# apache/datafusion

Hardware: AMD Instinct MI355X
Metric: tpch_q3_hash_join_rows_per_sec (higher is better)
Workload: dtype int64 keys / decimal128 payload; 1 GPU; INNER hash-join orders⋈lineitem on o_orderkey, TPC-H SF100, Q3 payload (o_orderdate,o_shippriority,l_orderkey,l_extendedprice,l_discount), device-resident inputs; build_rows=150000000, probe_rows=599960064, output_rows=599960064, join_table=rank_map, probe=single_pass_unordered, parallelism=single GPU, exchange=none

## Files before the change

datafusion_amd/csrc/internal.hpp:

```cpp
#pragma once
#include <atomic>
#include <hip/hip_runtime.h>

#include <chrono>
#include <cstdint>
#include <cstring>
#include <map>
#include <memory>
#include <mutex>
#include <stdexcept>
#include <string>
#include <thread>
#include <vector>

#include "../../include/dfgpu.h"

namespace dfgpu {

struct Error : std::runtime_error {
  using std::runtime_error::runtime_error;
};

void set_last_error(const std::string& msg);

// ... 79 lines not shown

  bool profiling = false;
  struct Rec {
    std::string name;
    hipEvent_t a, b;
    int64_t bytes;
    std::thread::id thread;
  };
  std::map<std::thread::id, int64_t> kernel_ns_by_thread;
  std::vector<Rec> recs;
  std::vector<dfgpu_kernel_stat> stats;
  struct Launch { int stat; float ms; int64_t bytes; };
  std::vector<Launch> launches;
  void collect();
};

Runtime& rt();
void scan_upload_caches_drop(int device);
int64_t scan_upload_caches_bytes(int device);
Runtime& rt_of(int device);
void use_device(int device);
int current_device();
const std::vector<int>& initialised_devices();
void require_init();

struct ProfileScope {
  hipEvent_t a = nullptr, b = nullptr;
  const char* name;
  int64_t bytes;
  ProfileScope(const char* name, int64_t algorithmic_bytes);
  ~ProfileScope();
};

struct DevBuf {
  void* ptr = nullptr;
  size_t bytes = 0;
  Runtime* owner = nullptr;
  std::shared_ptr<void> foreign;
  std::atomic<uint64_t> hint{0};
  std::atomic<uint64_t> all_hit_hint{0};
  explicit DevBuf(size_t n);
  DevBuf(void* p, size_t n, std::shared_ptr<void> keep_alive) : ptr(p), bytes(n), foreign(std::move(keep_alive)) {}
  ~DevBuf();
  DevBuf(const DevBuf&) = delete;
  DevBuf& operator=(const DevBuf&) = delete;
  template <typename T>
  T* as() const { return reinterpret_cast<T*>(ptr); }
};
using BufPtr = std::shared_ptr<DevBuf>;
inline BufPtr make_buf(size_t bytes) { return std::make_shared<DevBuf>(bytes ? bytes : 1); }
BufPtr make_zero_buf(size_t bytes);

void d2h(void* dst, const void* src, size_t n);
extern std::atomic<int64_t> g_pinned_driver_allocs, g_pinned_driver_ns;
void* pinned_alloc(size_t n);
void pinned_release(void* p);
void* stage_alloc(size_t n);
template <class T> struct StageAllocator {
  using value_type = T;
  StageAllocator() = default;
  template <class U> StageAllocator(const StageAllocator<U>&) {}
  T* allocate(size_t n) { return static_cast<T*>(stage_alloc(n * sizeof(T))); }
  void deallocate(T* p, size_t) { pinned_release(p); }
  template <class U> void construct(U* p) noexcept { ::new ((void*)p) U; }
  template <class U, class... A> void construct(U* p, A&&... a) { ::new ((void*)p) U(std::forward<A>(a)...); }
  template <class U> bool operator==(const StageAllocator<U>&) const { return true; }
  template <class U> bool operator!=(const StageAllocator<U>&) const { return false; }
};
template <class T> using StageVec = std::vector<T, StageAllocator<T>>;
struct PinnedBuf {
  void* ptr = nullptr;
  size_t bytes = 0;
  explicit PinnedBuf(size_t n) : ptr(pinned_alloc(n ? n : 1)), bytes(n) {}
  ~PinnedBuf() { pinned_release(ptr); }
  PinnedBuf(const PinnedBuf&) = delete;
  PinnedBuf& operator=(const PinnedBuf&) = delete;
  template <class T> T* as() const { return reinterpret_cast<T*>(ptr); }
};
void h2d_async(void* dst, const void* src, size_t n);

inline int type_width(int t) {
  switch (t) {
    case DFGPU_INT32: case DFGPU_UINT32: case DFGPU_DATE32: return 4;
    case DFGPU_INT64: case DFGPU_UINT64: case DFGPU_FLOAT64: return 8;
    case DFGPU_DECIMAL128: return 16;
    case DFGPU_UINT8: return 1;
    case DFGPU_BOOL: return 0;
    case DFGPU_UTF8:
      throw Error("a Utf8 column reached an operator that works on fixed-width columns: dictionary-encode it first (dfgpu_table_dictionary_encode)");
  }
  throw Error("unknown dfgpu_type " + std::to_string(t));
}
inline size_t bitmap_bytes(int64_t n) { return (size_t)((n + 63) / 64) * 8; }
inline size_t data_bytes(int t, int64_t n) { return t == DFGPU_BOOL ? bitmap_bytes(n) : (size_t)n * type_width(t); }
inline bool is_integer_like(int t) {
  return t == DFGPU_INT32 || t == DFGPU_INT64 || t == DFGPU_UINT8 || t == DFGPU_UINT32 || t == DFGPU_UINT64 || t == DFGPU_DATE32;
}
inline bool is_signed_type(int t) { return t == DFGPU_INT32 || t == DFGPU_INT64 || t == DFGPU_DATE32 || t == DFGPU_DECIMAL128; }
std::string type_name(const dfgpu_field& f);

struct ColStats {
  long long min = 0, max = 0;
  int64_t valid = 0;
  bool ascending = false;
  bool nondecreasing = false;
  bool has_present = false;
// ... 144 lines not shown
```

datafusion_amd/csrc/join.hip:

```cpp
#include <thread>
#include <functional>
#include <cstdlib>

#include "device.hpp"
#include "internal.hpp"
#include "grouped.hpp"

namespace dfgpu {

Table compact_table(const Table& in, const std::vector<int>& cols, const uint64_t* mask, const uint64_t* mask_valid);
void pack_bytes_to_bitmap(const uint8_t* bytes, int64_t n, uint64_t* words);

enum TableKind : int { KIND_HASH = 0, KIND_ARRAY = 1, KIND_RANK = 2, KIND_RADIX = 3, KIND_FLAT = 4, KIND_FLAT16 = 5,
                       KIND_RETURNED = 6 };
template <int KIND> constexpr bool kind_is_flat() { return KIND == KIND_FLAT || KIND == KIND_FLAT16; }
template <int KIND> constexpr bool kind_is_direct() { return KIND == KIND_ARRAY || KIND == KIND_RANK; }

struct FlatLayout {
  int n;
  uint8_t off[MAX_KEYS];
  uint8_t width[MAX_KEYS];
  int8_t null_bit[MAX_KEYS];
};
constexpr double RANK_MAP_MIN_KEY_DENSITY = 1.0 / 256.0;
// ... 253 lines not shown
      }
    }
    return;
  }
  const int64_t stride = (int64_t)gridDim.x * BLOCK;
  for (int64_t i0 = (int64_t)blockIdx.x * BLOCK + threadIdx.x; i0 < n; i0 += stride * BUILD_UNROLL) {
    uint64_t lo[BUILD_UNROLL];
    bool ok[BUILD_UNROLL];
#pragma unroll
    for (int j = 0; j < BUILD_UNROLL; j++) {
      int64_t i = i0 + j * stride;
      lo[j] = load_key<KT>(k, i < n ? i : n - 1);
    }
#pragma unroll
    for (int j = 0; j < BUILD_UNROLL; j++) {
      int64_t i = i0 + j * stride;
      ok[j] = i < n;
      if (HASV) ok[j] = ok[j] && bit_at(k.valid, i < n ? i : n - 1);
    }
#pragma unroll
    for (int j = 0; j < BUILD_UNROLL; j++) {
      if (!ok[j]) continue;
      const uint64_t idx = lo[j] - offset;
      const unsigned long long bit = 1ull << (idx & 63);
      (void)__hip_atomic_fetch_or(&bits[idx >> 6], bit, __ATOMIC_RELAXED, __HIP_MEMORY_SCOPE_AGENT);
    }
  }
}
typedef unsigned long long rt_u64x2 __attribute__((ext_vector_type(2)));
typedef unsigned rt_u32x4 __attribute__((ext_vector_type(4)));
template <int KT>
__device__ __forceinline__ void load_keys4(const KeyCol& k, int64_t i0, uint64_t (&out)[4]) {
  if (KT == KT_I64 && ((uintptr_t)k.data & 15) == 0) {
    const rt_u64x2* p = reinterpret_cast<const rt_u64x2*>((const uint64_t*)k.data + i0);
    const rt_u64x2 a = __builtin_nontemporal_load(p), b = __builtin_nontemporal_load(p + 1);
    out[0] = a.x; out[1] = a.y; out[2] = b.x; out[3] = b.y;
  } else if ((KT == KT_I32 || KT == KT_U32) && ((uintptr_t)k.data & 15) == 0) {
    const rt_u32x4 a = __builtin_nontemporal_load(reinterpret_cast<const rt_u32x4*>((const uint32_t*)k.data + i0));
    out[0] = KT == KT_I32 ? (uint64_t)(int64_t)(int32_t)a.x : a.x;
    out[1] = KT == KT_I32 ? (uint64_t)(int64_t)(int32_t)a.y : a.y;
    out[2] = KT == KT_I32 ? (uint64_t)(int64_t)(int32_t)a.z : a.z;
    out[3] = KT == KT_I32 ? (uint64_t)(int64_t)(int32_t)a.w : a.w;
  } else {
#pragma unroll
    for (int j = 0; j < 4; j++) out[j] = load_key<KT, true>(k, i0 + j);
  }
}
constexpr int RT_ROWS = 4096;
constexpr int RT_WIN = 1024;
constexpr int RT_LANE_ROWS = 4;
constexpr int RT_CHUNK = WAVE * RT_LANE_ROWS;
constexpr int RT_STEPS = RT_ROWS / RT_CHUNK / (BLOCK / WAVE);
template <int KT, bool VERIFY>
__global__ __launch_bounds__(BLOCK) void k_rank_tab_onepass(KeyCol k, int64_t n, uint64_t offset, uint64_t range, ulonglong2* __restrict__ tab, int* __restrict__ flag) {
  __shared__ unsigned long long s_bits[RT_WIN];
  __shared__ unsigned s_first[RT_WIN];
  constexpr int WAVES = BLOCK / WAVE;
  const unsigned lane = lane_id();
  const int wv = threadIdx.x >> 6;
  const int64_t r0 = (int64_t)blockIdx.x * RT_ROWS;
  const int64_t r1 = r0 + RT_ROWS < n ? r0 + RT_ROWS : n;
  const uint64_t n_words = (range >> 6) + 1;
  uint64_t idx[RT_STEPS][RT_LANE_ROWS], pidx[RT_STEPS];
#pragma unroll
  for (int c = 0; c < RT_STEPS; c++) {
    const int64_t i0 = r0 + (int64_t)(c * WAVES + wv) * RT_CHUNK + lane * RT_LANE_ROWS;
    if (i0 + RT_LANE_ROWS <= n) {
      load_keys4<KT>(k, i0, idx[c]);
#pragma unroll
      for (int j = 0; j < RT_LANE_ROWS; j++) idx[c][j] -= offset;
    } else {
#pragma unroll
      for (int j = 0; j < RT_LANE_ROWS; j++) idx[c][j] = load_key<KT, true>(k, i0 + j < n ? i0 + j : n - 1) - offset;
    }
    pidx[c] = 0;
    if (VERIFY) pidx[c] = load_key<KT>(k, i0 < n ? (i0 > 0 ? i0 - 1 : 0) : n - 1) - offset;
  }
  const bool tail_lane = wv == WAVES - 1 && r1 + lane < n;
  const uint64_t tail_idx = tail_lane ? load_key<KT>(k, r1 + lane) - offset : ~0ull;
  const uint64_t w_first = r0 > 0 ? ((load_key<KT>(k, r0 - 1) - offset) >> 6) + 1 : 0ull;
  const uint64_t w_last = (load_key<KT>(k, r1 - 1) - offset) >> 6;
  const uint64_t w_end = w_last < n_words ? w_last : n_words - 1;
  const int cnt = w_end < w_first ? 0 : (w_end - w_first + 1 < (uint64_t)RT_WIN ? (int)(w_end - w_first + 1) : RT_WIN);
  for (int t = threadIdx.x; t < cnt; t += BLOCK) {
    s_bits[t] = 0ull;
    s_first[t] = ~0u;
  }
  __syncthreads();
  auto put = [&](uint64_t w, unsigned long long bits, int64_t row, bool first_known, bool is_first) {
    const uint64_t slot = w - w_first;
    if (slot < (uint64_t)cnt) {
      atomicOr(&s_bits[slot], bits);
      atomicMin(&s_first[slot], (unsigned)(row - r0));
    } else {
      unsigned long long* e = reinterpret_cast<unsigned long long*>(tab + w);
      (void)__hip_atomic_fetch_or(e, bits, __ATOMIC_RELAXED, __HIP_MEMORY_SCOPE_AGENT);
      if (!first_known) is_first = row == 0 || ((load_key<KT>(k, row - 1) - offset) >> 6) != w;
      if (is_first) e[1] = (unsigned long long)row;
    }
  };
#pragma unroll
  for (int c = 0; c < RT_STEPS; c++) {
    const int64_t i0 = r0 + (int64_t)(c * WAVES + wv) * RT_CHUNK + lane * RT_LANE_ROWS;
    bool ok[RT_LANE_ROWS], later[RT_LANE_ROWS];
    uint64_t w = ~0ull, v = 0ull;
    unsigned rel = 0;
    bool found = false, bad = false, any_later = false;
#pragma unroll
    for (int j = 0; j < RT_LANE_ROWS; j++) {
      const uint64_t x = idx[c][j];
      if (VERIFY) bad = bad || (i0 + j < r1 && (x > range || (i0 + j > 0 && x <= (j ? idx[c][j - 1] : pidx[c]))));
      ok[j] = i0 + j < r1 && x <= range && (x >> 6) >= w_first;
      if (ok[j] && !found) {
        found = true;
        w = x >> 6;
        rel = (unsigned)(i0 + j - r0);
      }
      const bool lead = ok[j] && (x >> 6) == w;
      v |= lead ? 1ull << (x & 63) : 0ull;
      later[j] = ok[j] && !lead;
      any_later = any_later || later[j];
    }
    if (VERIFY && ballot64(bad) != 0 && lane == 0) atomicOr(flag, 1);
    const uint64_t inc = wave_inclusive_sum_dpp(v);
    const uint64_t w_next = __shfl_down(w, 1, 64);
    const uint64_t tails = ballot64(lane == 63 || w_next != w);
    const uint64_t heads = (tails << 1) | 1ull;
    const int head_lane = 63 - __builtin_clzll(heads & ((2ull << lane) - 1ull));
    const uint64_t before = __shfl(inc - v, head_lane, 64);
    const unsigned head_rel = __shfl(rel, head_lane, 64);
    if (found && ((tails >> lane) & 1ull)) put(w, inc - before, r0 + head_rel, false, false);
    if (any_later) {
#pragma unroll
      for (int j = 1; j < RT_LANE_ROWS; j++)
        if (later[j]) put(idx[c][j] >> 6, 1ull << (idx[c][j] & 63), i0 + j, true, (idx[c][j - 1] >> 6) != (idx[c][j] >> 6));
    }
  }
  if (tail_lane && tail_idx <= range && (tail_idx >> 6) == w_last && w_last >= w_first) put(w_last, 1ull << (tail_idx & 63), r1 + lane, true, false);
  __syncthreads();
// ... 859 lines not shown
        s_prefix = excl;
        s_full = agg == (uint64_t)TILE_WORDS * 64;
      }
    }
    __syncthreads();
    uint64_t wave_base = s_prefix;
#pragma unroll
    for (int i = 0; i < BLOCK / WAVE; i++)
      if (i < wv) wave_base += s_wcount[i];

    const bool full = s_full;
    for (int cidx = 0; cidx < cols.n; cidx++) {
      const int width = cols.width[cidx];
      const bool from_build = cidx < cols.n_build;
      const bool stream = full && !from_build;
      uint64_t ob = wave_base;
#pragma unroll
      for (int j = 0; j < W; j++) {
        const int64_t d = (int64_t)(ob + mbcnt(word[j]));
        ob += (uint32_t)__popcll(word[j]);
        if (!((word[j] >> lane) & 1ull)) continue;
        if (KEYREG && cidx == cols.key_col) {
          if (KT == KT_I64) reinterpret_cast<uint64_t*>(cols.dst[cidx])[d] = key[KEYREG ? j : 0];
          else if (KT == KT_U8) reinterpret_cast<uint8_t*>(cols.dst[cidx])[d] = (uint8_t)key[KEYREG ? j : 0];
          else reinterpret_cast<uint32_t*>(cols.dst[cidx])[d] = (uint32_t)key[KEYREG ? j : 0];
          continue;
        }
        int64_t s = from_build ? (int64_t)m[j] - 1 : ((w0 + j) << 6) + lane;
        if (KIND == KIND_RETURNED && from_build) {
          if (rec_in_regs) {
            const uint4 rv = rec16[KIND == KIND_RETURNED ? j : 0];
            const int bo = cols.ret_add[cidx] * width;
            const uint32_t w32 = (bo >> 2) == 1 ? rv.y : (bo >> 2) == 2 ? rv.z : rv.w;
            if (width == 4) reinterpret_cast<uint32_t*>(cols.dst[cidx])[d] = w32;
            else if (width == 8) reinterpret_cast<uint64_t*>(cols.dst[cidx])[d] = ((uint64_t)rv.w << 32) | rv.z;
            else reinterpret_cast<uint8_t*>(cols.dst[cidx])[d] = (uint8_t)(w32 >> ((bo & 3) * 8));
            continue;
          }
          s = (int64_t)c.ret_dest[((w0 + j) << 6) + lane] * cols.ret_mul[cidx] + cols.ret_add[cidx];
        }
        switch (width) {
          case 16: jcopy_stream<uint4>(cols.src[cidx], cols.dst[cidx], s, d, stream, full); break;
          case 8: jcopy_stream<uint64_t>(cols.src[cidx], cols.dst[cidx], s, d, stream, full); break;
          case 4: jcopy_stream<uint32_t>(cols.src[cidx], cols.dst[cidx], s, d, stream, full); break;
          case 1: jcopy_stream<uint8_t>(cols.src[cidx], cols.dst[cidx], s, d, stream, full); break;
        }
      }
    }
    if (!ORDERED) return;
    __syncthreads();
  }
}

constexpr int SHARED_W = 8;
template <int KIND, int KT, int W>
__global__ __launch_bounds__(BLOCK) void k_join_probe_shared(ProbeCtx c, JoinCopyCols cols, int64_t np, FusedCtl* __restrict__ ctl) {
  static_assert(W % 4 == 0, "4-byte columns leave four words (256 rows) at a time");
  const int64_t n_words = (np + 63) >> 6;
  const unsigned lane = lane_id();
  const int64_t w0 = ((((int64_t)blockIdx.x * BLOCK) + threadIdx.x) >> 6) * W;
  if (w0 >= n_words) return;
  uint32_t m[W];
  lookup_words<KIND, KT, W>(c, w0, np, m);
  bool missed = false;
#pragma unroll
  for (int j = 0; j < W; j++) missed |= (((w0 + j) << 6) + lane) < np && m[j] == 0;
  const uint64_t miss_word = ballot64(missed);
  if (miss_word && lane == (unsigned)__builtin_ctzll(miss_word)) ctl->ticket = 1u;
  for (int cidx = 0; cidx < cols.n_build; cidx++) {
    const int width = cols.width[cidx];
    if (width == 4) {
#pragma unroll
      for (int g = 0; g < W / 4; g++) {
        uint32_t v[4], o[4];
#pragma unroll
        for (int jj = 0; jj < 4; jj++) {
          const int j = 4 * g + jj;
          const bool live = (((w0 + j) << 6) + lane) < np && m[j];
          v[jj] = live ? reinterpret_cast<const uint32_t*>(cols.src[cidx])[m[j] - 1] : 0u;
        }
        const int word_of_lane = lane >> 4;
#pragma unroll
        for (int q = 0; q < 4; q++) {
          const int from = (4 * lane + q) & 63;
#pragma unroll
          for (int jj = 0; jj < 4; jj++) {
            const uint32_t t = __shfl(v[jj], from);
            if (jj == word_of_lane) o[q] = t;
          }
        }
        const int64_t row0 = ((w0 + 4 * g) << 6) + 4 * (int64_t)lane;
        uint32_t* dst = reinterpret_cast<uint32_t*>(cols.dst[cidx]) + row0;
        if (row0 + 3 < np) {
          stream_store(reinterpret_cast<uint4*>(dst), make_uint4(o[0], o[1], o[2], o[3]));
        } else {
#pragma unroll
          for (int q = 0; q < 4; q++)
            if (row0 + q < np) dst[q] = o[q];
        }
      }
      continue;
    }
#pragma unroll
    for (int j = 0; j < W; j++) {
      const int64_t d = ((w0 + j) << 6) + lane;
      if (d >= np || !m[j]) continue;
      const int64_t s = (int64_t)m[j] - 1;
      switch (width) {
        case 16: jcopy_stream<uint4>(cols.src[cidx], cols.dst[cidx], s, d, false, true); break;
        case 8: jcopy_stream<uint64_t>(cols.src[cidx], cols.dst[cidx], s, d, false, true); break;
        case 1: jcopy_stream<uint8_t>(cols.src[cidx], cols.dst[cidx], s, d, false, true); break;
      }
    }
  }
}

constexpr int EL_WORDS = 128;
constexpr int EL_WORDS_SPARSE = 1024;
constexpr int EL_CAP = 8192;
template <int KIND, int KT, int EW>
__global__ __launch_bounds__(BLOCK) void k_join_emit_listed(ProbeCtx c, JoinCopyCols cols, int64_t np, const uint64_t* __restrict__ out_words,
// ... 673 lines not shown
      MinMax res;
      d2h(&res, mm->ptr, sizeof res);
      n_valid_keys = (int64_t)res.valid;
      if (res.valid > 0) {
        range = (uint64_t)res.smax - (uint64_t)res.smin;
        have_stats = range != UINT64_MAX;
        kmin = res.smin;
        ascending = res.unsorted == 0;
        std::atomic_store(&const_cast<Column&>(kc).stats, std::make_shared<ColStats>(ColStats{res.smin, res.smax, (int64_t)res.valid, res.unsorted == 0, res.descends == 0}));
      }
    }
  }
  const double dense = have_stats ? (double)nb / ((double)range + 1.0) : 0.0;
  bool am_ok = have_stats && !(range >= (uint64_t)opts.perfect_hash_join_small_build_threshold && dense <= opts.perfect_hash_join_min_key_density);
  if (opts.table_mode == 2) am_ok = have_stats;
  am_ok = am_ok && range < (1ull << 34);
  bool rank_ok = have_stats && (opts.table_mode == 0 || opts.table_mode == 3) && range < (1ull << 40) &&
                 (range < (uint64_t)opts.perfect_hash_join_small_build_threshold || dense >= RANK_MAP_MIN_KEY_DENSITY || opts.table_mode == 3);
  DFGPU_CHECK(!speculated || rank_ok, "internal: speculative build statistics outside the rank map's gate");
  DFGPU_CHECK(!(opts.table_mode == 2 && !am_ok), "direct-address join table requested but not applicable");
  DFGPU_CHECK(!(opts.table_mode == 3 && !rank_ok), "rank-map join table requested but not applicable");
  constexpr int64_t MALL_BYTES = (int64_t)256 << 20;

  BufPtr flag;
  auto need_flag = [&]() {
    if (!flag) flag = make_zero_buf(4);
    return flag->as<int>();
  };
  int dup = 0;
  bool flat_wide = false;
  if (rank_ok && !ascending && !speculated && opts.table_mode == 0 && opts.probe_mode == 4 && ks.n == 1 && nb * 8 > MALL_BYTES && nb >= ((int64_t)1 << 22)) {
    const int64_t m = (int64_t)1 << 18;
    const uint64_t slots = (uint64_t)1 << 20;
    BufPtr table = make_zero_buf((size_t)slots * 8);
    {
      ProfileScope ps("join_build_sample_duplicates", m * 2 * ks.c[0].width);
      with_key_type(ks.c[0].type, [&](auto kt) {
        k_sample_duplicates<decltype(kt)::value><<<grid_for(2 * m, BLOCK), BLOCK, 0, r.stream>>>(ks.c[0], nb, nb / m, m, table->as<unsigned long long>(), slots - 1, need_flag());
      });
      DFGPU_HIP(hipGetLastError());
    }
    int seen = 0;
    d2h(&seen, need_flag(), 4);
    if (seen) {
      dup = 1;
      rank_ok = false;
      DFGPU_HIP(hipMemsetAsync(need_flag(), 0, 4, r.stream));
    }
  }
  if (rank_ok) {
    const int64_t n_words = (int64_t)(range >> 6) + 1;
    BufPtr eager_tab;
    if (ascending && (double)nb >= 0.15 * ((double)range + 1.0)) {
      eager_tab = make_zero_buf((size_t)n_words * 16);
      ProfileScope ps("join_build_rank_tab_onepass", nb * ks.c[0].width + n_words * 16);
      const int g = (int)((nb + RT_ROWS - 1) / RT_ROWS);
      with_key_type(ks.c[0].type, [&](auto kt) {
        constexpr int T = decltype(kt)::value;
        if (speculated) k_rank_tab_onepass<T, true><<<g, BLOCK, 0, r.stream>>>(ks.c[0], nb, (uint64_t)kmin, range, eager_tab->as<ulonglong2>(), need_flag());
        else k_rank_tab_onepass<T, false><<<g, BLOCK, 0, r.stream>>>(ks.c[0], nb, (uint64_t)kmin, range, eager_tab->as<ulonglong2>(), nullptr);
      });
      DFGPU_HIP(hipGetLastError());
    } else {
    jt->rank_bits = make_zero_buf((size_t)n_words * 8);
    {
      ProfileScope ps("join_build_rank_map", nb * ks.c[0].width);
      int g = std::min(grid_for(nb, BLOCK * BUILD_UNROLL), 2048);
      unsigned long long* bits = jt->rank_bits->as<unsigned long long>();
      KeyCol kc0 = ks.c[0];
      BufPtr grouped_keys;
      constexpr int RB_BITS = 10;
      const bool lds_bits = !ascending && nb > (1 << 22) && n_words * 8 > ((int64_t)16 << 20) && (range >> RB_BITS) < (1ull << 20) - 64;
      if (lds_bits) {
        const GroupSpec gs = group_spec((uint64_t)kmin, range + 1, 1 << RB_BITS);
        GroupedRows gr = group_rows_by_key(kc0, nb, gs, RB_BITS, nullptr, true, false, {}, {}, "join_build_group_keys");
        const int P = 1 << RB_BITS;
        std::vector<uint64_t> gfirst((size_t)P + 1);
        uint64_t max_span = 0;
        for (int q = 0; q <= P; q++) {
          const unsigned __int128 v = ((((unsigned __int128)(unsigned)q) << 64) + gs.mul - 1) / gs.mul;
          gfirst[(size_t)q] = v > (unsigned __int128)(range + 1) || q == P ? range + 1 : (uint64_t)v;
          if (q) max_span = std::max(max_span, gfirst[(size_t)q] - gfirst[(size_t)q - 1]);
        }
        BufPtr d_first = make_buf(gfirst.size() * 8);
        h2d_async(d_first->ptr, gfirst.data(), gfirst.size() * 8);
        const size_t lds = (size_t)((max_span >> 6) + 2) * 8;
        DFGPU_HIP(hipFuncSetAttribute(reinterpret_cast<const void*>(k_rank_bits_grouped), hipFuncAttributeMaxDynamicSharedMemorySize, (int)lds));
        k_rank_bits_grouped<<<P, RB_THREADS, lds, r.stream>>>(gr.keys->as<uint64_t>(), gr.bounds->as<uint64_t>(), d_first->as<uint64_t>(), (uint64_t)kmin, bits, need_flag());
        DFGPU_HIP(hipGetLastError());
        DFGPU_HIP(hipStreamSynchronize(r.stream));
      } else {
      if (!ascending && !kc0.valid && kc0.width == 8 && nb > (1 << 22) && n_words * 8 > ((int64_t)16 << 20)) {
        const Column& kcol = build.cols[(size_t)key_cols[0]];
        grouped_keys = kcol.data;
        if (kcol.data_offset != 0) {
          grouped_keys = make_buf((size_t)nb * 8);
          DFGPU_HIP(hipMemcpyAsync(grouped_keys->ptr, kcol.ptr(), (size_t)nb * 8, hipMemcpyDeviceToDevice, r.stream));
        }
        int range_bits = 0;
        while (range_bits < 64 && ((range + 1) >> range_bits)) range_bits++;
        radix_group_keys(grouped_keys, nb, std::max(0, range_bits - 6), 6);
        kc0.data = grouped_keys->ptr;
      }
      const bool byte_map = !ascending && nb > (1 << 20) && range < (1ull << 32);
      if (byte_map) {
        BufPtr bytes = make_zero_buf((size_t)n_words * 64);
        with_key_type(kc0.type, [&](auto kt) {
          constexpr int T = decltype(kt)::value;
          if (kc0.valid) k_rank_setbytes<T, true><<<g, BLOCK, 0, r.stream>>>(kc0, nb, (uint64_t)kmin, bytes->as<uint8_t>());
          else k_rank_setbytes<T, false><<<g, BLOCK, 0, r.stream>>>(kc0, nb, (uint64_t)kmin, bytes->as<uint8_t>());
        });
        DFGPU_HIP(hipGetLastError());
        pack_bytes_to_bitmap(bytes->as<uint8_t>(), n_words * 64, jt->rank_bits->as<uint64_t>());
// ... 596 lines not shown
    grouped.device = probe.device;
    Column gk = kc;
    gk.data = keys;
    gk.data_offset = 0;
    gk.length = n_grouped;
    gk.stats.reset();
    grouped.cols.push_back(std::move(gk));
    in_grouped_probe = true;
    Table res;
    try {
      res = join_probe(jt, grouped, {0}, join_type, bout_in, {0}, nullptr, nullptr);
    } catch (...) {
      in_grouped_probe = false;
      throw;
    }
    in_grouped_probe = false;
    std::lock_guard<std::mutex> lk(jt.mu);
    jt.info.probe_rows -= n_grouped;
    return res;
  }
  if (fused_ok && fused_mode == FUSED_UNORDERED && np > (1 << 22) && !unclustered && !in_grouped_probe && !returned) {
    int64_t row_bytes = key_bytes / std::max<int64_t>(np, 1) + out_row_bytes;
    for (int c : pout) {
      bool is_key = false;
      for (int k : pk) is_key |= k == c;
      if (!is_key) row_bytes += type_width(probe.cols[c].field.type);
    }
    if (row_bytes * (FUSED_W * BLOCK) < 12 * 6000) fused_mode = FUSED_PLACED;
  }
  const bool one_match_path = np > 0 && (probe_side_only || fast_inner);
  const bool use_fused_now = use_fused;
  const bool pred_in_counts = lazy != nullptr && use_fused && listed && fused_mode == FUSED_PLACED && !returned && (kind == KIND_RANK || kind == KIND_ARRAY);
  if (!pred_in_counts) need_mask();
  if (row_mask || pred_in_counts) {
    DFGPU_CHECK(mask_consumed != nullptr, "probe row mask without a fallback");
    *mask_consumed = use_fused || one_match_path;
    if (!*mask_consumed) return Table{};
    ctx.row_mask = row_mask;
  }
  const bool listed_flavour = use_fused_now && listed && fused_mode == FUSED_PLACED && kind == KIND_RANK;
  if (!listed_flavour) need_tab();
  if (use_fused_now && fused_mode != FUSED_PLACED) {
    size_t free_b = 0, total_b = 0;
    DFGPU_HIP(hipMemGetInfo(&free_b, &total_b));
    DFGPU_CHECK(np * out_row_bytes <= (int64_t)free_b + r.cached, "single-pass probe: the np-row upper bound of the output does not fit in HBM");
  }

  if (use_fused_now) {
    const int64_t tile_words = (int64_t)FUSED_W * (BLOCK / WAVE);
    const int64_t n_tiles = (n_words + tile_words - 1) / tile_words;
    const int invert = join_type == DFGPU_JOIN_RIGHT_ANTI;
    ctx.row_mask = row_mask;
    BufPtr state = fused_mode == FUSED_LOOKBACK ? make_zero_buf((size_t)n_tiles * 8) : nullptr;
    BufPtr ctl = make_zero_buf(sizeof(FusedCtl));
    BufPtr out_words;
    int64_t n_alloc = np;
    static thread_local bool no_speculation = false;
    DevBuf* hit_hint = nullptr;
    uint64_t hit_tag = 0;
    auto probe_again_counted = [&](hipEvent_t ea, hipEvent_t eb) {
      if (hit_hint) hit_hint->all_hit_hint.store(hit_tag, std::memory_order_relaxed);
      if (r.profiling) {
        std::lock_guard<std::mutex> lk(r.mu);
        r.recs.push_back(Runtime::Rec{"join_probe_speculation_missed", ea, eb, 0, std::this_thread::get_id()});
      }
      {
        std::lock_guard<std::mutex> lk(jt.mu);
        jt.info.probe_rows -= np;
      }
      out = Table{};
      no_speculation = true;
      Table again;
      try {
        again = join_probe(jt, probe, pk, join_type, bout_in, pout, row_mask, mask_consumed);
      } catch (...) {
        no_speculation = false;
        throw;
      }
      no_speculation = false;
      return again;
    };
    bool speculate = false;
    const bool spec_kind = kind == KIND_RANK || kind == KIND_ARRAY || kind == KIND_FLAT || kind == KIND_FLAT16;
    const bool may_sample = !row_mask && !lazy && !invert && !no_speculation && spec_kind && np >= option_int("join.share_probe_min_rows", 1 << 22);
    const bool share_wanted = option_on("join.share_probe", true) && jt.probe_mode != 2 && !returned && (fast_inner || join_type == DFGPU_JOIN_RIGHT_SEMI);
    if (returned_all_hit && !no_speculation) {
      speculate = true;
    } else if (may_sample && (share_wanted || (fused_mode == FUSED_PLACED && !listed))) {
      hit_hint = probe.cols[(size_t)pk[0]].data.get();
      hit_tag = all_hit_tag(jt, probe, pk, kind);
      const uint64_t h = hit_hint->all_hit_hint.load(std::memory_order_relaxed);
      if ((h & ~1ull) == hit_tag) {
        speculate = (h & 1ull) != 0;
      } else {
        constexpr int S = 1024;
        BufPtr miss = make_zero_buf(4);
        with_kind_and_key(kind, ctx.pkeys.c[0].type, [&](auto kd, auto kt) {
          k_sample_all_hit<decltype(kd)::value, decltype(kt)::value><<<S * WAVE / BLOCK, BLOCK, 0, r.stream>>>(ctx, np, std::max<int64_t>(1, n_words / S), S, miss->as<int>());
        });
        DFGPU_HIP(hipGetLastError());
        int m = 0;
        d2h(&m, miss->ptr, 4);
        speculate = m == 0;
        hit_hint->all_hit_hint.store(hit_tag | (speculate ? 1ull : 0ull), std::memory_order_relaxed);
      }
    }
    if (speculate && share_wanted && !returned_all_hit) {
      need_tab();
      JoinCopyCols jc{};
      jc.key_col = -1;
      int64_t bytes = key_bytes;
      for (int c : bout) {
        const Column& sc = jt.build.cols[c];
        out.cols.push_back(alloc_like(sc, np));
        jc.src[jc.n] = sc.ptr();
        jc.dst[jc.n] = out.cols.back().data->ptr;
        jc.width[jc.n] = type_width(sc.field.type);
        bytes += (jt.build.nrows + np) * jc.width[jc.n];
        jc.n++;
      }
      jc.n_build = jc.n;
      hipEvent_t ea = nullptr, eb = nullptr, sa = nullptr, sb = nullptr;
      if (r.profiling) {
        for (hipEvent_t* e : {&ea, &eb, &sa, &sb}) DFGPU_HIP(hipEventCreate(e));
        DFGPU_HIP(hipEventRecord(ea, r.stream));
      }
      with_kind_and_key(kind, ctx.pkeys.c[0].type, [&](auto kd, auto kt) {
        constexpr int K = decltype(kd)::value, T = decltype(kt)::value;
        if constexpr (K == KIND_RANK || K == KIND_ARRAY || K == KIND_FLAT || K == KIND_FLAT16) {
          const int64_t waves = (n_words + SHARED_W - 1) / SHARED_W;
          const unsigned g = (unsigned)((waves + BLOCK / WAVE - 1) / (BLOCK / WAVE));
          k_join_probe_shared<K, T, SHARED_W><<<g, BLOCK, 0, r.stream>>>(ctx, jc, np, ctl->as<FusedCtl>());
        }
      });
      DFGPU_HIP(hipGetLastError());
      if (r.profiling) {
        DFGPU_HIP(hipEventRecord(eb, r.stream));
        DFGPU_HIP(hipEventRecord(sa, r.stream));
        DFGPU_HIP(hipEventRecord(sb, r.stream));
      }
      unsigned missed = 0;
      d2h(&missed, &ctl->as<FusedCtl>()->ticket, 4);
      if (missed) {
        if (r.profiling) {
          DFGPU_HIP(hipEventDestroy(sa));
          DFGPU_HIP(hipEventDestroy(sb));
        }
        return probe_again_counted(ea, eb);
      }
      for (int c : pout) {
        out.cols.push_back(probe.cols[c]);
        out.cols.back().length = np;
      }
      if (r.profiling) {
        std::lock_guard<std::mutex> lk(r.mu);
        r.recs.push_back(Runtime::Rec{want_single ? "join_probe_fused" : "join_probe_placed", ea, eb, bytes, std::this_thread::get_id()});
        r.recs.push_back(Runtime::Rec{"join_probe_shared_columns", sa, sb, 0, std::this_thread::get_id()});
      }
      out.nrows = np;
      jt.info.output_rows += out.nrows;
      return out;
    }
    speculate = speculate && fused_mode == FUSED_PLACED && !listed;
    if (fused_mode == FUSED_PLACED && !speculate) {
      BufPtr counts = make_buf((size_t)n_tiles * 4);
      state = make_buf((size_t)(n_tiles + 1) * 8);
      if (listed) out_words = make_buf((size_t)n_words * 8);
      if (kind == KIND_RANK) need_bits();
      {
        ProfileScope ps("join_probe_tile_counts", key_bytes + (pred_in_counts ? np * lazy->pred_bytes_per_row : 0));
        with_kind_and_key(kind, ctx.pkeys.c[0].type, [&](auto kd, auto kt) {
          constexpr int K = decltype(kd)::value, T = decltype(kt)::value;
          if constexpr (kind_is_direct<K>()) {
            const bool nt = option_on("join.counts_nt", true);
            if (pred_in_counts) {
              if (nt) k_join_tile_counts<K, T, FUSED_W, true, true><<<(unsigned)n_tiles, BLOCK, 0, r.stream>>>(ctx, np, invert, nullptr, counts->as<uint32_t>(), out_words->as<uint64_t>(), lazy->pred);
              else k_join_tile_counts<K, T, FUSED_W, true><<<(unsigned)n_tiles, BLOCK, 0, r.stream>>>(ctx, np, invert, nullptr, counts->as<uint32_t>(), out_words->as<uint64_t>(), lazy->pred);
              return;
            }
            if (nt) {
              k_join_tile_counts<K, T, FUSED_W, false, true><<<(unsigned)n_tiles, BLOCK, 0, r.stream>>>(ctx, np, invert, row_mask, counts->as<uint32_t>(), out_words ? out_words->as<uint64_t>() : nullptr);
              return;
            }
          }
          k_join_tile_counts<K, T, FUSED_W><<<(unsigned)n_tiles, BLOCK, 0, r.stream>>>(
              ctx, np, invert, row_mask, counts->as<uint32_t>(), out_words ? out_words->as<uint64_t>() : nullptr);
        });
        DFGPU_HIP(hipGetLastError());
      }
      scan_u32(counts->as<uint32_t>(), n_tiles, state->as<uint64_t>());
      n_alloc = (int64_t)read_u64(state->as<uint64_t>() + n_tiles);
      listed = listed && n_alloc * 4 <= np;
      if (!listed) need_tab();
      if (pred_in_counts && !listed) {
        row_mask = out_words->as<uint64_t>();
        ctx.row_mask = row_mask;
      }
    }
    JoinCopyCols jc{};
    jc.key_col = -1;
    int64_t bytes_in = key_bytes, bytes_per_out = 0, bytes_build_once = 0;
    for (int c : bout) {
      const Column& sc = jt.build.cols[c];
      out.cols.push_back(alloc_like(sc, n_alloc));
      jc.src[jc.n] = sc.ptr();
      jc.dst[jc.n] = out.cols.back().data->ptr;
      jc.width[jc.n] = type_width(sc.field.type);
      if (returned) {
        jc.src[jc.n] = rp.rec->ptr;
        jc.ret_mul[jc.n] = rp.mul[(size_t)jc.n];
        jc.ret_add[jc.n] = rp.add[(size_t)jc.n];
      }
      bytes_per_out += jc.width[jc.n];
      bytes_build_once += jt.build.nrows * jc.width[jc.n];
      jc.n++;
    }
    jc.n_build = jc.n;
    for (int c : pout) {
      const Column& sc = probe.cols[c];
      out.cols.push_back(alloc_like(sc, n_alloc));
      jc.src[jc.n] = sc.ptr();
      jc.dst[jc.n] = out.cols.back().data->ptr;
      jc.width[jc.n] = type_width(sc.field.type);
      bool is_key = false;
      for (int k : pk) is_key |= k == c;
      if (!is_key) bytes_in += np * jc.width[jc.n];
      if (is_key && (kind == KIND_ARRAY || kind == KIND_RANK) && pk.size() == 1 && jc.key_col < 0 && !sc.validity) jc.key_col = jc.n;
      bytes_per_out += jc.width[jc.n];
      jc.n++;
    }
    hipEvent_t ea = nullptr, eb = nullptr;
    if (r.profiling) {
      DFGPU_HIP(hipEventCreate(&ea));
      DFGPU_HIP(hipEventCreate(&eb));
      DFGPU_HIP(hipEventRecord(ea, r.stream));
    }
    int64_t n_out = n_alloc;
    if (fused_mode != FUSED_PLACED || n_alloc > 0) {
      const unsigned g = fused_mode == FUSED_LOOKBACK ? (unsigned)std::min<int64_t>(n_tiles, (int64_t)r.num_cus * 8) : (unsigned)n_tiles;
      uint64_t* st = state ? state->as<uint64_t>() : nullptr;
      auto launch = [&](auto kern) { kern<<<g, BLOCK, 0, r.stream>>>(ctx, jc, np, invert, st, ctl->as<FusedCtl>(), row_mask); };
      with_kind_and_key(kind, ctx.pkeys.c[0].type, [&](auto kd, auto kt) {
        constexpr int K = decltype(kd)::value, T = decltype(kt)::value;
        constexpr bool KR = kind_is_direct<K>();
        if constexpr (KR) {
          if (listed) {
            const int64_t den = option_int("join.listed_sparse_den", 32);
            if (den > 0 && n_alloc * den <= np) {
              const int64_t groups = (n_words + EL_WORDS_SPARSE - 1) / EL_WORDS_SPARSE;
              k_join_emit_listed<K, T, EL_WORDS_SPARSE><<<(unsigned)groups, BLOCK, 0, r.stream>>>(ctx, jc, np, out_words->as<uint64_t>(), st, (int)(EL_WORDS_SPARSE / tile_words));
            } else {
              const int64_t groups = (n_words + EL_WORDS - 1) / EL_WORDS;
              k_join_emit_listed<K, T, EL_WORDS><<<(unsigned)groups, BLOCK, 0, r.stream>>>(ctx, jc, np, out_words->as<uint64_t>(), st, (int)(EL_WORDS / tile_words));
            }
            return;
          }
        }
        if (fused_mode == FUSED_LOOKBACK) launch(k_join_probe_fused<K, T, FUSED_W, FUSED_LOOKBACK, false>);
        else if (fused_mode == FUSED_PLACED) {
          if (KR && jc.key_col >= 0) launch(k_join_probe_fused<K, T, FUSED_W, FUSED_PLACED, KR>);
          else launch(k_join_probe_fused<K, T, FUSED_W, FUSED_PLACED, false>);
        } else {
          if (KR && jc.key_col >= 0) launch(k_join_probe_fused<K, T, FUSED_W, FUSED_UNORDERED, KR>);
          else launch(k_join_probe_fused<K, T, FUSED_W, FUSED_UNORDERED, false>);
        }
      });
      DFGPU_HIP(hipGetLastError());
      if (r.profiling) DFGPU_HIP(hipEventRecord(eb, r.stream));
      if (fused_mode != FUSED_PLACED) n_out = (int64_t)read_u64(reinterpret_cast<const uint64_t*>(&ctl->as<FusedCtl>()->total));
      if (speculate) {
        unsigned missed = 0;
        d2h(&missed, &ctl->as<FusedCtl>()->ticket, 4);
        if (missed) return probe_again_counted(ea, eb);
      }
    } else if (r.profiling) {
      DFGPU_HIP(hipEventRecord(eb, r.stream));
    }
    if (r.profiling) {
      std::lock_guard<std::mutex> lk(r.mu);
      r.recs.push_back(Runtime::Rec{listed ? "join_probe_listed" : fused_mode == FUSED_PLACED ? "join_probe_placed" : "join_probe_fused", ea, eb,
                                    bytes_in + (n_out > 0 ? bytes_build_once : 0) + n_out * bytes_per_out, std::this_thread::get_id()});
    }
    out.nrows = n_out;
    for (Column& c : out.cols) c.length = n_out;
  } else if (np > 0 && (probe_side_only || (build_side_only && jt.keys_unique) || fast_inner)) {
    BufPtr mask = make_buf(bitmap_bytes(np));
    BufPtr first = fast_inner ? make_buf((size_t)np * 4) : nullptr;
    {
      ProfileScope ps("join_probe_lookup", key_bytes);
      int g = grid_for(n_words, (BLOCK / WAVE) * PROBE_UNROLL);
      int invert = join_type == DFGPU_JOIN_RIGHT_ANTI;
      with_kind_and_key(jt.kind, ctx.pkeys.c[0].type, [&](auto kd, auto kt) {
        k_probe_first<decltype(kd)::value, decltype(kt)::value><<<g, BLOCK, 0, r.stream>>>(ctx, np, invert, first ? first->as<uint32_t>() : nullptr,
                                                                                           mask->as<uint64_t>(), visited);
// ... 807 lines not shown
```

datafusion_amd/csrc/runtime.hip:

```cpp
#include "internal.hpp"

#include <chrono>
#include <algorithm>
#include <cstring>
#include <atomic>

namespace dfgpu {

static thread_local std::string g_last_error;
void set_last_error(const std::string& msg) { g_last_error = msg; }

static std::mutex g_devices_mu;
static std::vector<std::unique_ptr<Runtime>> g_runtimes;
static std::vector<int> g_initialised;
static Runtime g_uninitialised;
static thread_local int t_device = -1;
static thread_local int t_hip_device = -1;

const std::vector<int>& initialised_devices() { return g_initialised; }
int current_device() {
  if (t_device >= 0) return t_device;
  return g_initialised.empty() ? -1 : g_initialised[0];
}
Runtime& rt_of(int device) {
// ... 230 lines not shown
    live.erase(it);
    in_use -= (int64_t)cap;
    if (!g_multi_thread.load(std::memory_order_seq_cst)) {
      free_blocks.emplace(cap, p);
      cached += (int64_t)cap;
      return;
    }
  }
  thread_device(device).pending.emplace_back(cap, p);
}

void Runtime::trim() {
  scan_upload_caches_drop(device);
  call_epilogue();
  std::multimap<size_t, void*> blocks;
  {
    std::lock_guard<std::mutex> lk(mu);
    blocks.swap(free_blocks);
    cached = 0;
  }
  if (blocks.empty()) return;
  (void)hipDeviceSynchronize();
  for (auto& kv : blocks) (void)hipFree(kv.second);
}

DevBuf::DevBuf(size_t n) : bytes(n), owner(&rt()) { ptr = owner->alloc(n); }
DevBuf::~DevBuf() {
  if (owner) owner->free(ptr);
}

BufPtr make_zero_buf(size_t bytes) {
  BufPtr b = make_buf(bytes);
  DFGPU_HIP(hipMemsetAsync(b->ptr, 0, bytes ? bytes : 1, rt().stream));
  return b;
}

void d2h(void* dst, const void* src, size_t n) {
  constexpr size_t PIN = 64 << 10;
  static thread_local void* t_pin = nullptr;
  if (n <= PIN && option_on("runtime.pinned_readback", true)) {
    if (!t_pin && hipHostMalloc(&t_pin, PIN, hipHostMallocDefault) != hipSuccess) {
      (void)hipGetLastError();
      t_pin = nullptr;
    }
    if (t_pin) {
      DFGPU_HIP(hipMemcpyAsync(t_pin, src, n, hipMemcpyDeviceToHost, rt().stream));
      DFGPU_HIP(hipStreamSynchronize(rt().stream));
      std::memcpy(dst, t_pin, n);
      return;
    }
  }
  DFGPU_HIP(hipMemcpyAsync(dst, src, n, hipMemcpyDeviceToHost, rt().stream));
  DFGPU_HIP(hipStreamSynchronize(rt().stream));
}
void h2d_async(void* dst, const void* src, size_t n) {
  DFGPU_HIP(hipMemcpyAsync(dst, src, n, hipMemcpyHostToDevice, rt().stream));
}
uint64_t read_u64(const uint64_t* dev) {
  uint64_t v = 0;
  d2h(&v, dev, 8);
  return v;
}

dfgpu_metrics& thread_metrics() {
  static thread_local dfgpu_metrics m{};
  return m;
}

ProfileScope::ProfileScope(const char* n, int64_t algorithmic_bytes) : name(n), bytes(algorithmic_bytes) {
  Runtime& r = rt();
  thread_metrics().hbm_bytes_algorithmic += algorithmic_bytes;
  if (!r.profiling) return;
  (void)hipEventCreate(&a);
  (void)hipEventCreate(&b);
  (void)hipEventRecord(a, r.stream);
}
ProfileScope::~ProfileScope() {
  if (!a) return;
  Runtime& r = rt();
  (void)hipEventRecord(b, r.stream);
  std::lock_guard<std::mutex> lk(r.mu);
  r.recs.push_back({name, a, b, bytes, std::this_thread::get_id()});
}

void Runtime::collect() {
  if (recs.empty()) return;
  (void)hipDeviceSynchronize();
  for (auto& rec : recs) {
    float ms = 0.f;
    (void)hipEventElapsedTime(&ms, rec.a, rec.b);
    (void)hipEventDestroy(rec.a);
    (void)hipEventDestroy(rec.b);
    auto it = std::find_if(stats.begin(), stats.end(), [&](const dfgpu_kernel_stat& s) { return rec.name == s.name; });
    if (it == stats.end()) {
      dfgpu_kernel_stat s{};
      std::strncpy(s.name, rec.name.c_str(), sizeof(s.name) - 1);
      stats.push_back(s);
      it = stats.end() - 1;
    }
    it->calls += 1;
    it->total_ms += ms;
    it->algorithmic_bytes += rec.bytes;
    if (launches.size() >= 65536) launches.erase(launches.begin(), launches.begin() + 32768);
    launches.push_back(Launch{(int)(it - stats.begin()), ms, rec.bytes});
    kernel_ns_by_thread[rec.thread] += (int64_t)((double)ms * 1e6);
  }
// ... 312 lines not shown
```

Measured before the change: 340.5 billion rows/s.

## Skip rank-table zero fill and signal probe misses via epoch flag

```diff
diff --git a/datafusion_amd/csrc/internal.hpp b/datafusion_amd/csrc/internal.hpp
--- a/datafusion_amd/csrc/internal.hpp
+++ b/datafusion_amd/csrc/internal.hpp
@@ -155,6 +155,13 @@
 BufPtr make_zero_buf(size_t bytes);
 
 void d2h(void* dst, const void* src, size_t n);
+struct EpochFlag {
+  unsigned* dev;
+  unsigned* host_dev;
+  const volatile unsigned* host;
+  unsigned epoch;
+};
+bool next_epoch_flag(EpochFlag& f);
 extern std::atomic<int64_t> g_pinned_driver_allocs, g_pinned_driver_ns;
 void* pinned_alloc(size_t n);
 void pinned_release(void* p);
diff --git a/datafusion_amd/csrc/join.hip b/datafusion_amd/csrc/join.hip
--- a/datafusion_amd/csrc/join.hip
+++ b/datafusion_amd/csrc/join.hip
@@ -329,7 +329,8 @@
 constexpr int RT_CHUNK = WAVE * RT_LANE_ROWS;
 constexpr int RT_STEPS = RT_ROWS / RT_CHUNK / (BLOCK / WAVE);
 template <int KT, bool VERIFY>
-__global__ __launch_bounds__(BLOCK) void k_rank_tab_onepass(KeyCol k, int64_t n, uint64_t offset, uint64_t range, ulonglong2* __restrict__ tab, int* __restrict__ flag) {
+__global__ __launch_bounds__(BLOCK) void k_rank_tab_onepass(KeyCol k, int64_t n, uint64_t offset, uint64_t range, ulonglong2* __restrict__ tab, int* __restrict__ flag,
+                                                            int tab_zeroed) {
   __shared__ unsigned long long s_bits[RT_WIN];
   __shared__ unsigned s_first[RT_WIN];
   constexpr int WAVES = BLOCK / WAVE;
@@ -362,6 +363,14 @@
   for (int t = threadIdx.x; t < cnt; t += BLOCK) {
     s_bits[t] = 0ull;
     s_first[t] = ~0u;
+  }
+  if (!VERIFY && !tab_zeroed) {
+    const bool last_wg = blockIdx.x == gridDim.x - 1;
+    const uint64_t z0 = w_first + (uint64_t)cnt, z1 = last_wg ? n_words : w_end + 1;
+    if (z0 < z1) {
+      for (uint64_t t = z0 + threadIdx.x; t < z1; t += BLOCK) tab[t] = make_ulonglong2(0ull, 0ull);
+      __threadfence();
+    }
   }
   __syncthreads();
   auto put = [&](uint64_t w, unsigned long long bits, int64_t row, bool first_known, bool is_first) {
@@ -1327,9 +1336,26 @@
   }
 }
 
+struct MissFlag {
+  unsigned* dev;
+  unsigned* host;
+  unsigned epoch;
+};
+__device__ __forceinline__ void raise_miss(const MissFlag& f, uint64_t miss_word, unsigned lane) {
+  if (!miss_word || lane != (unsigned)__builtin_ctzll(miss_word)) return;
+  if (!f.host) {
+    *f.dev = f.epoch;
+    return;
+  }
+  if (__hip_atomic_load(f.dev, __ATOMIC_RELAXED, __HIP_MEMORY_SCOPE_AGENT) != f.epoch) {
+    __hip_atomic_store(f.dev, f.epoch, __ATOMIC_RELAXED, __HIP_MEMORY_SCOPE_AGENT);
+    __hip_atomic_store(f.host, f.epoch, __ATOMIC_RELAXED, __HIP_MEMORY_SCOPE_SYSTEM);
+  }
+}
+
 constexpr int SHARED_W = 8;
 template <int KIND, int KT, int W>
-__global__ __launch_bounds__(BLOCK) void k_join_probe_shared(ProbeCtx c, JoinCopyCols cols, int64_t np, FusedCtl* __restrict__ ctl) {
+__global__ __launch_bounds__(BLOCK) void k_join_probe_shared(ProbeCtx c, JoinCopyCols cols, int64_t np, MissFlag flag) {
   static_assert(W % 4 == 0, "4-byte columns leave four words (256 rows) at a time");
   const int64_t n_words = (np + 63) >> 6;
   const unsigned lane = lane_id();
@@ -1341,7 +1367,7 @@
 #pragma unroll
   for (int j = 0; j < W; j++) missed |= (((w0 + j) << 6) + lane) < np && m[j] == 0;
   const uint64_t miss_word = ballot64(missed);
-  if (miss_word && lane == (unsigned)__builtin_ctzll(miss_word)) ctl->ticket = 1u;
+  raise_miss(flag, miss_word, lane);
   for (int cidx = 0; cidx < cols.n_build; cidx++) {
     const int width = cols.width[cidx];
     if (width == 4) {
@@ -2121,13 +2147,14 @@
     const int64_t n_words = (int64_t)(range >> 6) + 1;
     BufPtr eager_tab;
     if (ascending && (double)nb >= 0.15 * ((double)range + 1.0)) {
-      eager_tab = make_zero_buf((size_t)n_words * 16);
+      const bool no_fill = !speculated && option_on("join.onepass_no_fill", true);
+      eager_tab = no_fill ? make_buf((size_t)n_words * 16) : make_zero_buf((size_t)n_words * 16);
       ProfileScope ps("join_build_rank_tab_onepass", nb * ks.c[0].width + n_words * 16);
       const int g = (int)((nb + RT_ROWS - 1) / RT_ROWS);
       with_key_type(ks.c[0].type, [&](auto kt) {
         constexpr int T = decltype(kt)::value;
-        if (speculated) k_rank_tab_onepass<T, true><<<g, BLOCK, 0, r.stream>>>(ks.c[0], nb, (uint64_t)kmin, range, eager_tab->as<ulonglong2>(), need_flag());
-        else k_rank_tab_onepass<T, false><<<g, BLOCK, 0, r.stream>>>(ks.c[0], nb, (uint64_t)kmin, range, eager_tab->as<ulonglong2>(), nullptr);
+        if (speculated) k_rank_tab_onepass<T, true><<<g, BLOCK, 0, r.stream>>>(ks.c[0], nb, (uint64_t)kmin, range, eager_tab->as<ulonglong2>(), need_flag(), 1);
+        else k_rank_tab_onepass<T, false><<<g, BLOCK, 0, r.stream>>>(ks.c[0], nb, (uint64_t)kmin, range, eager_tab->as<ulonglong2>(), nullptr, no_fill ? 0 : 1);
       });
       DFGPU_HIP(hipGetLastError());
     } else {
@@ -2830,7 +2857,11 @@
     const int invert = join_type == DFGPU_JOIN_RIGHT_ANTI;
     ctx.row_mask = row_mask;
     BufPtr state = fused_mode == FUSED_LOOKBACK ? make_zero_buf((size_t)n_tiles * 8) : nullptr;
-    BufPtr ctl = make_zero_buf(sizeof(FusedCtl));
+    BufPtr ctl;
+    auto need_ctl = [&]() {
+      if (!ctl) ctl = make_zero_buf(sizeof(FusedCtl));
+      return ctl->as<FusedCtl>();
+    };
     BufPtr out_words;
     int64_t n_alloc = np;
     static thread_local bool no_speculation = false;
@@ -2903,12 +2934,15 @@
         for (hipEvent_t* e : {&ea, &eb, &sa, &sb}) DFGPU_HIP(hipEventCreate(e));
         DFGPU_HIP(hipEventRecord(ea, r.stream));
       }
+      EpochFlag ef{};
+      const bool epoch_flag = next_epoch_flag(ef);
+      const MissFlag mf = epoch_flag ? MissFlag{ef.dev, ef.host_dev, ef.epoch} : MissFlag{&need_ctl()->ticket, nullptr, 1u};
       with_kind_and_key(kind, ctx.pkeys.c[0].type, [&](auto kd, auto kt) {
         constexpr int K = decltype(kd)::value, T = decltype(kt)::value;
         if constexpr (K == KIND_RANK || K == KIND_ARRAY || K == KIND_FLAT || K == KIND_FLAT16) {
           const int64_t waves = (n_words + SHARED_W - 1) / SHARED_W;
           const unsigned g = (unsigned)((waves + BLOCK / WAVE - 1) / (BLOCK / WAVE));
-          k_join_probe_shared<K, T, SHARED_W><<<g, BLOCK, 0, r.stream>>>(ctx, jc, np, ctl->as<FusedCtl>());
+          k_join_probe_shared<K, T, SHARED_W><<<g, BLOCK, 0, r.stream>>>(ctx, jc, np, mf);
         }
       });
       DFGPU_HIP(hipGetLastError());
@@ -2918,7 +2952,12 @@
         DFGPU_HIP(hipEventRecord(sb, r.stream));
       }
       unsigned missed = 0;
-      d2h(&missed, &ctl->as<FusedCtl>()->ticket, 4);
+      if (epoch_flag) {
+        DFGPU_HIP(hipStreamSynchronize(r.stream));
+        missed = *ef.host == ef.epoch;
+      } else {
+        d2h(&missed, &ctl->as<FusedCtl>()->ticket, 4);
+      }
       if (missed) {
         if (r.profiling) {
           DFGPU_HIP(hipEventDestroy(sa));
@@ -3017,7 +3056,7 @@
     if (fused_mode != FUSED_PLACED || n_alloc > 0) {
       const unsigned g = fused_mode == FUSED_LOOKBACK ? (unsigned)std::min<int64_t>(n_tiles, (int64_t)r.num_cus * 8) : (unsigned)n_tiles;
       uint64_t* st = state ? state->as<uint64_t>() : nullptr;
-      auto launch = [&](auto kern) { kern<<<g, BLOCK, 0, r.stream>>>(ctx, jc, np, invert, st, ctl->as<FusedCtl>(), row_mask); };
+      auto launch = [&](auto kern) { kern<<<g, BLOCK, 0, r.stream>>>(ctx, jc, np, invert, st, need_ctl(), row_mask); };
       with_kind_and_key(kind, ctx.pkeys.c[0].type, [&](auto kd, auto kt) {
         constexpr int K = decltype(kd)::value, T = decltype(kt)::value;
         constexpr bool KR = kind_is_direct<K>();
diff --git a/datafusion_amd/csrc/runtime.hip b/datafusion_amd/csrc/runtime.hip
--- a/datafusion_amd/csrc/runtime.hip
+++ b/datafusion_amd/csrc/runtime.hip
@@ -306,6 +306,45 @@
   }
   DFGPU_HIP(hipMemcpyAsync(dst, src, n, hipMemcpyDeviceToHost, rt().stream));
   DFGPU_HIP(hipStreamSynchronize(rt().stream));
+}
+bool next_epoch_flag(EpochFlag& f) {
+  if (!option_on("runtime.pinned_readback", true)) return false;
+  struct Words {
+    unsigned* dev = nullptr;
+    unsigned* host = nullptr;
+    unsigned* host_dev = nullptr;
+    unsigned epoch = 0;
+    bool refused = false;
+  };
+  static thread_local std::map<int, Words> t_words;
+  Runtime& r = rt();
+  Words& w = t_words[r.device];
+  if (w.refused) return false;
+  if (!w.host) {
+    void *h = nullptr, *hd = nullptr, *d = nullptr;
+    const bool ok = hipHostMalloc(&h, 64, hipHostMallocDefault) == hipSuccess && hipHostGetDevicePointer(&hd, h, 0) == hipSuccess && hipMalloc(&d, 64) == hipSuccess &&
+                    hipMemsetAsync(d, 0, 64, r.stream) == hipSuccess && hipStreamSynchronize(r.stream) == hipSuccess;
+    if (!ok) {
+      (void)hipGetLastError();
+      if (h) (void)hipHostFree(h);
+      if (d) (void)hipFree(d);
+      w.refused = true;
+      return false;
+    }
+    *static_cast<volatile unsigned*>(h) = 0u;
+    w.host = static_cast<unsigned*>(h);
+    w.host_dev = static_cast<unsigned*>(hd);
+    w.dev = static_cast<unsigned*>(d);
+  }
+  if (++w.epoch == 0) {
+    DFGPU_HIP(hipStreamSynchronize(r.stream));
+    DFGPU_HIP(hipMemsetAsync(w.dev, 0, 4, r.stream));
+    DFGPU_HIP(hipStreamSynchronize(r.stream));
+    *static_cast<volatile unsigned*>(w.host) = 0u;
+    w.epoch = 1;
+  }
+  f = EpochFlag{w.dev, w.host_dev, w.host, w.epoch};
+  return true;
 }
 void h2d_async(void* dst, const void* src, size_t n) {
   DFGPU_HIP(hipMemcpyAsync(dst, src, n, hipMemcpyHostToDevice, rt().stream));
```

New measurement: 344.0 billion rows/s, median of 4. About the same (+1.0%).
